# zengxianyu/sketchedit

Hardware: AMD Instinct MI355X
Metric: images/sec (higher is better)
Workload: dtype f32; 1 GPU; SketchEdit inference forward (netM+netG, use_cam, pool max) 256x256 batch 32 per GPU, procedural weights; global_batch=32, size=256, per_gpu_batch=32, execution=default, two streams

## Files before the change

### sketchedit_amd/_lib.py

```python
import contextlib
import ctypes
import os
import subprocess
import threading

import numpy as np

_HERE = os.path.dirname(os.path.abspath(__file__))
LIB_PATH = os.environ.get("SKETCHEDIT_HIP_LIB") or os.path.join(_HERE, "lib", "libsketchedit_hip.so")
CSRC = os.path.join(_HERE, "csrc")
SOURCES = ["se_gconv.hip", "se_rconv16.hip", "se_rconv96.hip", "se_rtile.hip", "se_rtilew.hip", "se_wino.hip", "se_wino24.hip", "se_wino48.hip", "se_wino_up.hip", "se_wino_up48.hip", "se_attention.hip", "se_att_stream.hip", "se_misc.hip", "se_resize.hip",
           "se_window.hip", "se_feather.hip", "se_fill.hip", "se_select.hip", "se_lasso.hip", "se_modify.hip", "se_outline.hip", "se_move.hip", "se_warp.hip", "se_filter.hip", "se_adjust.hip", "se_png.hip", "se_jpg.hip", "se_pack.hip",
           "se_plan.hip", "se_api_window.hip", "se_api_select.hip", "se_api_move.hip", "se_api_codec.hip", "se_api_debug.hip", "se_api.hip"]

SE_NET_G, SE_NET_M = 0, 1
RESAMPLE_LANCZOS, RESAMPLE_BILINEAR, RESAMPLE_BICUBIC = 1, 2, 3
FLAG_USE_CAM, FLAG_POOL_MAX, FLAG_NO_MASK_CC, FLAG_NO_MASK_COARSE, FLAG_JOINT_TRAIN_INP = 1, 2, 4, 8, 16
FLAG_LOW_LATENCY, FLAG_GRAPH, FLAG_PACKED_OUT, FLAG_BF16, FLAG_CONSERVATIVE = 32, 64, 128, 256, 512
LOW_LATENCY_MAX_PIXELS = 3 * 256 * 256
LOW_LATENCY_MAX_SINGLE_IMAGE = 512 * 512

SYMBOLS = ["se_create", "se_destroy", "se_last_error", "se_version", "se_load_weights", "se_weights_ready",
           "se_workspace_bytes", "se_netM_forward", "se_netM_forward_ex", "se_netG_forward", "se_netG_forward_taps", "se_inference", "se_inference_u8", "se_gated_conv2d",
           "se_gated_conv2d_ex", "se_attention", "se_attention_ex", "se_quantize_u8", "se_dequantize_u8", "se_inference_u8io", "se_profile_enable",
           "se_profile_report", "se_debug_set_option", "se_debug_get_option", "se_debug_reset_options", "se_debug_gconv_form",
           "se_resize_u8", "se_prepare_u8", "se_edit_u8", "se_edit_u8_workspace_bytes", "se_resample_coeffs",
# ... 317 lines not shown
    load_library().se_debug_reset_options()


def gconv_form(cin, cout, H, W, k=3, stride=1, rate=1, act="elu", upsample=False, cin1=0, x1_is_vector=False, B=1,
               low_latency=False, bf16=False, conservative=False, net=SE_NET_G):
    flags = (FLAG_LOW_LATENCY if low_latency else 0) | (FLAG_BF16 if bf16 else 0) | (FLAG_CONSERVATIVE if conservative else 0)
    buf = ctypes.create_string_buffer(64)
    fn = load_library().se_debug_gconv_form
    fn.argtypes, fn.restype = [ctypes.c_int] * 14 + [ctypes.c_char_p, ctypes.c_size_t], ctypes.c_int
    if fn(cin, cin1, int(bool(x1_is_vector)), cout, k, stride, rate, {"elu": 0, "relu": 1, None: 2}[act],
          int(bool(upsample)), B, H, W, flags, net, buf, len(buf)):
        raise SketchEditHipError("gconv_form: not a layer gated_conv2d takes")
    return buf.value.decode().split(",")


def pair_rule(B, H, W, low_latency=False):
    v = ctypes.c_int(-1)
    name = "SE_PAIR_RULE:%d,%d,%d,%d" % (B, H, W, FLAG_LOW_LATENCY if low_latency else 0)
    if load_library().se_debug_get_option(name.encode(), ctypes.byref(v)):
        raise SketchEditHipError("pair_rule: bad shape B=%d H=%d W=%d" % (B, H, W))
    return bool(v.value)


def flags_from_opt(opt):
    f = 0
    if getattr(opt, "use_cam", False):
        f |= FLAG_USE_CAM
    pool = getattr(opt, "pool_type", "avg")
    if pool == "max":
        f |= FLAG_POOL_MAX
# ... 1096 lines not shown
```

### sketchedit_amd/csrc/se_api_debug.hip

```cpp
#include "se_host.h"

using namespace se;

extern "C" {

int se_profile_enable(se_ctx* c, int on) {
  if (!c) return 1;
  std::lock_guard<std::mutex> lk(c->mu);
  HIPCHK(c, hipSetDevice(c->device));
  c->prof.recs.clear();
  c->prof.used = 0;
  if (on && c->prof.pool.empty()) {
    c->prof.pool.resize(2 * 1024);
    for (auto& e : c->prof.pool) HIPCHK(c, hipEventCreate(&e));
  }
  c->prof.on = on != 0;
  return 0;
}

int se_profile_report(se_ctx* c, char* buf, size_t cap) {
  if (!c || !buf || cap < 64) return 1;
  std::lock_guard<std::mutex> lk(c->mu);
  HIPCHK(c, hipSetDevice(c->device));
  HIPCHK(c, hipDeviceSynchronize());
// ... 44 lines not shown
    first = false;
  }
  s += "]}";
  if (s.size() + 1 > cap) return fail(c, "profile buffer too small");
  memcpy(buf, s.c_str(), s.size() + 1);
  return 0;
}

int se_debug_set_option(const char* name, int value) { return opt_set(name, value); }
int se_debug_get_option(const char* name, int* value) {
  static const char q[] = "SE_PAIR_RULE:";
  if (name && value && !strncmp(name, q, sizeof q - 1)) {
    int B = 0, H = 0, W = 0, flags = 0, end = 0;
    if (sscanf(name + sizeof q - 1, "%d,%d,%d,%d%n", &B, &H, &W, &flags, &end) != 4 || name[sizeof q - 1 + end] || B < 1 || H < 1 || W < 1) return 1;
    *value = pair_rule(B, H, W, flags) ? 1 : 0;
    return 0;
  }
  return opt_get(name, value);
}
void se_debug_reset_options(void) { opt_reset(); }

int se_debug_gconv_form(int cin, int cin1, int src1_is_vector, int cout, int k, int stride, int rate, int act, int upsample,
                        int B, int H, int W, int exec_flags, int net_id, char* out, size_t cap) {
  if (!out || cin <= 0 || cin1 < 0 || cout <= 0 || k <= 0 || stride <= 0 || rate <= 0 || B <= 0 || H <= 0 || W <= 0) return 1;
  const bool bf = (exec_flags & SE_FLAG_BF16) != 0;
  const int gran = bf ? 8 : 4;
  if (cin1 && ((cin % gran) || (cin1 % gran))) return 1;
  const LayerDef d = {"test", cin + cin1, cout, k, stride, rate, act, upsample};
  const bool raw = small_layer(d);
  if (raw && (k != 3 || cin != 12 || cin1 || (cout != 1 && cout != 3) || stride != 1 || rate != 1 || upsample)) return 1;
// ... 224 lines not shown
```

### sketchedit_amd/csrc/se_dispatch.h

```cpp
#pragma once
#include "se_kernels.h"

namespace se {

enum { ACT_ELU = 0, ACT_RELU = 1, ACT_NONE = 2 };

struct LayerDef {
  const char* name;
  int cin, cout, k, stride, rate, act, up;
};

inline bool small_layer(const LayerDef& d) { return d.act == ACT_NONE || d.cout == 3; }

struct ConvShape { int Ho, Wo, pad; };
inline ConvShape conv_shape(const LayerDef& d, int Hin, int Win) {
  const int pad = d.rate * (d.k - 1) / 2;
  if (d.up) return {2 * Hin, 2 * Win, pad};
  const int span = d.rate * (d.k - 1) + 1;
  return {(Hin + 2 * pad - span) / d.stride + 1, (Win + 2 * pad - span) / d.stride + 1, pad};
}

inline int choose_cfg(int G) {
  if (G <= 16) return GC_N24;
  if (G <= 24) return GC_N48;
// ... 3 lines not shown
}

inline bool rconv96_eligible(const LayerDef& d) {
  if (d.cout != 96 || d.rate != 1 || d.k != 3 || d.act == ACT_NONE) return false;
  if (d.stride == 2) return !d.up && d.cin == 24;
  if (d.stride != 1) return false;
  return d.up ? d.cin == 96 : (d.cin == 48 || d.cin == 24);
}

struct LayerFacts {
  bool small;
  int cfg, NP, G, T;
  int nch[2], CG[2];
  int dense, nchd;
  bool u, ub, u1, wv, wv16, u24, ub24, u24b, wx, wx2, wd, wdw, w16d, w16s, w96;
};

inline LayerFacts layer_facts(const LayerDef& d, int nchans) {
  LayerFacts f = {};
  f.cfg = -1;
  f.small = small_layer(d);
  if (f.small) return f;
  f.G = d.cout / 2;
  if (choose_cfg(f.G) < 0 || (f.G % 4)) return f;
  f.cfg = choose_cfg(f.G);
  f.NP = gconv_np(f.cfg);
  const int KW = d.up ? 2 : d.k;
  f.T = KW * KW;
  for (int bf = 0; bf < 2; ++bf) {
    const int per = bf ? 8 : 4, Cp = (nchans + per - 1) / per * per;
    f.CG[bf] = Cp / per;
    f.nch[bf] = (f.T * Cp + 8 * per - 1) / (8 * per);
  }
  const bool first = d.k == 5 && d.stride == 1 && d.rate == 1 && d.cout == 48;
  f.w16d = first && nchans >= 3 && nchans <= 4;
  f.wd = f.wdw = first && nchans >= 3 && nchans <= 5;
  f.dense = f.wd ? nchans : 0;
  f.nchd = (25 * f.dense + 31) / 32;
  f.w16s = d.k == 3 && d.stride == 1 && !d.up && (d.cin == 96 || d.cin == 192) && d.cout == 192;
  f.w96 = rconv96_eligible(d);
  if (d.k != 3 || d.stride != 1 || (nchans + 3) / 4 * 4 != d.cin) return f;
  if (d.up) {
    f.u = f.ub = (d.cin == 96 && d.cout == 96) || (d.cin == 48 && d.cout == 48);
  } else if ((d.cin == 96 || d.cin == 192) && d.cout == 192) {
    f.u = f.u24 = f.ub24 = true;
    f.u1 = f.wv = f.wv16 = f.u24b = d.cin == 192;
  } else if (d.cin == 48 && d.cout == 192) {
    f.u24 = f.ub24 = true;
  } else if (d.cin == 24 && d.cout == 24 && d.rate == 1) {
    f.wx = f.wx2 = true;
  } else if ((d.cin == 48 || d.cin == 24) && d.cout == 96) {
    f.u = f.ub = true;
  }
  return f;
}

enum { SRC2_NONE = 0, SRC2_TENSOR = 1, SRC2_VECTOR = 2 };
struct ConvCall {
  LayerDef def; LayerFacts facts;
  int B, Hin, Win, C0, C1;
  int src2;
  bool bf16, low_latency, conservative;
  int net;
  bool fold_scratch;
};

enum Form {
  F_SMALL_CONV, F_WINO, F_WINO24, F_WINO24_C48, F_WINO48, F_WINO48_C24, F_WINOUP, F_WINOUP48, F_RTILEW, F_RTILEW2,
  F_RTILE_DENSE5, F_RTILE_DENSE5W, F_RTILE_D4, F_RTILE, F_RCONV16, F_RCONV16_DUAL, F_RCONV96, F_GATHER
};
struct Choice {
  Form form;
  bool fold;
  bool wino_range;
};

inline bool magic_cg_ok(int CG, int nch) {
  const int m = (65536 + CG - 1) / CG;
  for (int gi = 0; gi < nch * 8 + 8; ++gi)
    if (((gi * m) >> 16) != gi / CG) return false;
  return true;
}
inline bool magic_kw_ok(int KW, int T) {
  const int m = 256 / KW + 1;
// ... 76 lines not shown
    const bool f43_net_ok = q.net == 0 || (f43_mode == 1 && !q.conservative);
    const bool f43 = (f43_mode == 1 || f43_mode == 2) && f43_net_ok && (s1 ? (!vec && f.u24b) : f.u24) && f.ub24 && (Win % (4 * d.rate)) == 0;
    return is(f43 ? F_WINO24 : F_WINO);
  }
  if (use_wino && f43_mode != 0 && !d.up && !two && C0 == 48 && d.cin == 48 && d.cout == 192 && d.stride == 1 && f.u24 && f.ub24 && fits96 &&
      (Hin % (2 * d.rate)) == 0 && (Win % (4 * d.rate)) == 0 && grid_ok(((long)(Hin / 2) * (Win / 4) + 31) / 32, min192))
    return is(F_WINO24_C48);
  if (use_wino && opt(OPT_WINOGRAD48) != 0 && !d.up && f.u && f.ub && !two && fits48 && even2 && grid_ok(wg64, min48)) {
    if (C0 == 48 && d.cin == 48) return is(F_WINO48);
    if (C0 == 24 && d.cin == 24 && d.cout == 96 && d.stride == 1) return is(F_WINO48_C24);
  }
  if (use_wino && opt(OPT_WINOGRAD_UP) != 0 && d.up && f.u && f.ub && !two && (Hin % 2) == 0 && (Win % 2) == 0 && grid_ok(4 * wg64, min48)) {
    if (C0 == 96 && d.cin == 96 && fits96) return is(F_WINOUP);
    if (opt(OPT_WINOGRAD_UP48) != 0 && C0 == 48 && d.cin == 48 && d.cout == 48 && fits48 && B * sh.Ho * sh.Wo * 96 < (1ll << 31)) return is(F_WINOUP48);
  }
  return is(choose_rtile(q));
}

inline const char* gconv_form_name(int cfg, bool small_grid, bool up2, bool two_src, bool bf16) {
#define SE_GF(n) n, n "_bf16", n "_2src", n "_2src_bf16", n "_up2", n "_up2_bf16", n "_up2_2src", n "_up2_2src_bf16"
#define SE_GS(n) { SE_GF(n), SE_GF(n "_small") }
  static const char* const names[4][16] = {SE_GS("gconv_n192"), SE_GS("gconv_n96"), SE_GS("gconv_n48"), SE_GS("gconv_n24")};
#undef SE_GS
#undef SE_GF
  if (cfg < 0 || cfg > 3) return nullptr;
  return names[cfg][(small_grid ? 8 : 0) | (up2 ? 4 : 0) | (two_src ? 2 : 0) | (bf16 ? 1 : 0)];
}

inline const char* form_name(const Choice& ch, const ConvCall& q) {
  const LayerDef& d = q.def;
// ... 3 lines not shown
    case F_WINO: return two ? "wino_2src" : "wino";
    case F_WINO24: return two ? "wino24_2src" : "wino24";
    case F_WINO24_C48: return "wino24_c48";
    case F_WINO48: return "wino48";
    case F_WINO48_C24: return "wino48_c24";
    case F_WINOUP: return "winoup";
    case F_WINOUP48: return "winoup48";
    case F_RTILEW: return "rtilew";
    case F_RTILEW2: return "rtilew2";
    case F_RTILE_DENSE5: return "rtile_dense5";
    case F_RTILE_DENSE5W: return "rtile_dense5w";
    case F_RTILE_D4: return "rtile_bf16_d4";
    case F_RTILE: return q.bf16 ? (d.up ? "rtile_bf16_up2" : "rtile_bf16") : (d.up ? "rtile_up2" : "rtile");
    case F_RCONV16: return "rconv16";
    case F_RCONV16_DUAL: return "rconv16_dual";
    case F_RCONV96: return d.up ? "rconv96_up" : d.stride == 2 ? "rconv96_s2" : q.C0 == 24 ? "rconv96_c24" : "rconv96";
    case F_GATHER: return gconv_form_name(q.facts.cfg, q.low_latency, d.up != 0, q.C0 / (q.bf16 ? 8 : 4) != q.facts.CG[q.bf16], q.bf16);
  }
  return nullptr;
}

}
```

### sketchedit_amd/csrc/se_kernels.h

```cpp
#pragma once
#include <hip/hip_runtime.h>
#include <stddef.h>
#include <stdint.h>

#include <vector>

struct se_window;

namespace se {

enum ProfLabel { PL_GCONV_N192 = 0, PL_GCONV_N96, PL_GCONV_N48, PL_GCONV_N24, PL_WINO_N192, PL_WINO_N96, PL_WINO_UP96, PL_SMALL_CONV, PL_PACK, PL_COLREDUCE,
                 PL_ATT_PREP, PL_ATT_SCORE, PL_ATT_SOFTMAX, PL_ATT_BOXSUM, PL_ATT_PV, PL_LAYOUT,
                 PL_ATT_STREAM_STATS, PL_ATT_STREAM_OUT, PL_RESIZE_H, PL_RESIZE_V, PL_WINDOW_GATHER, PL_WINDOW_BORDER, PL_WINDOW_PASTE,
                 PL_WINDOW_RESAMPLE_H, PL_WINDOW_PASTE_V, PL_WINDOW_SAVE, PL_WINDOW_SWAP, PL_WINDOW_LOCK_GATHER, PL_WINDOW_PASTE_LOCKED,
                 PL_WINDOW_PASTE_V_LOCKED, PL_SKETCH_TILES, PL_SKETCH_STROKES, PL_PNG_ROWS, PL_PNG_STRIPES,
                 PL_PNG_FINISH, PL_JPG_BLOCKS, PL_JPG_ROWS, PL_JPG_FINISH, PL_JPG2_BLOCKS, PL_JPG2_HIST, PL_JPG2_TABLES,
                 PL_WINDOW_PASTE_FEATHER, PL_FILL_MASKS, PL_FILL_KEEP, PL_SELECT_SIMILAR, PL_SELECT_FLOOD, PL_SELECT_GROW, PL_MODIFY_DISC, PL_MODIFY_VOTE,
                 PL_LASSO_FILL, PL_PLANE_COMBINE, PL_ADJUST, PL_HIST_TILES, PL_HIST_SUM, PL_ADJUST_LUT, PL_OUTLINE_COUNT, PL_OUTLINE_SCAN, PL_OUTLINE_EMIT, PL_FILTER_BLUR, PL_FILTER_MOSAIC, PL_MOVE_DROP,
                 PL_PLANE_SHIFT, PL_WARP_DROP, PL_PLANE_WARP, PL_COUNT };
const char* prof_label_name(int l);
struct Profiler {
  struct Rec { int label; const char* name; const char* form; double flops; double exec_flops; double bytes; long blocks; hipEvent_t a, b; };
  std::vector<Rec> recs;
  std::vector<hipEvent_t> pool;
// ... 5 lines not shown
void set_launch_grid(long blocks);
hipError_t ensure_max_lds(const void* func, int bytes);

#define SE_OPTIONS(X)                                                                                         \
  X(XCD_REMAP, 1)                                                             \
  X(RTILE, 1)                                              \
  X(RTILE_LL_MIN, 256)         \
  X(RTILE_WX, 2)          \
  X(RTILE_DENSE, 1)                                          \
  X(RTILE_D5W, 1)                                        \
  X(TEST_OFFSET_LIMIT, 0)  \
  X(TEST_POISON, 0)       \
  X(RCONV16, 1) X(RCONV16_DUAL, 1) X(RCONV96, 1) X(VECBIAS, 1)                                                  \
  X(WINOGRAD, 1) X(WINOGRAD48, 1) X(WINOGRAD_UP, 1) X(WINOGRAD_UP48, 1)                                         \
  X(WINOGRAD_F43, 1)      \
  X(GCONV_FAST, 1) X(FORK_DEFAULT, 1) X(LL_WINO_MIN_WG, 64) X(LL_WINO48_MIN_WG, 128)                            \
  X(ATT_FUSED, -1) X(ATT_FUSED_BF16, -1) X(ATT_PTILDE_LDS, 1) X(ATT_STATS_LDS, 1) X(ATT_E16, 1) X(ATT_SYM, 1)   \
  X(ATT_STREAM, 0)        \
  X(PAIR_MIN_PIXELS, 1 << 21)
enum Opt {
#define X(name, dflt) OPT_##name,
  SE_OPTIONS(X)
#undef X
  OPT_COUNT
};
int opt(int o);
int opt_set(const char* name, int value);
int opt_get(const char* name, int* value);
void opt_reset();
long long opt_epoch();
// ... 56 lines not shown
  int total_tiles;
  int act;
  int xcd;
  unsigned div_tpi_m, div_tw_m, div_d_m;
  int div_tpi_l, div_tw_l, div_d_l;
  const float* vbias;
};
hipError_t launch_wino(const WinoParams& p, hipStream_t st);
hipError_t launch_vecbias(const float* wv, const float* vec, float* T, int B, int C1, hipStream_t st, int round_vec = 0);
hipError_t launch_wino24(const WinoParams& p, hipStream_t st);
hipError_t launch_wino24_c48(const WinoParams& p, hipStream_t st);
hipError_t launch_wino48(const WinoParams& p, hipStream_t st);
hipError_t launch_wino48_c24(const WinoParams& p, hipStream_t st);
hipError_t launch_winoup(const WinoParams& p, hipStream_t st);
hipError_t launch_winoup48(const WinoParams& p, hipStream_t st);

struct RConvParams {
  const void* src;
  const void* wpk;
  const float* bias;
  void* dst;
  int B, h, w, d;
  int hs, ws;
  int ty, tx;
  int act;
  int xcd;
  const float* vbias;
  int dual;
};
hipError_t launch_rconv16(const RConvParams& p, hipStream_t st);
// ... 218 lines not shown
```

### sketchedit_amd/csrc/se_pack.h

```cpp
#pragma once
#include <hip/hip_runtime.h>

#include "se_dispatch.h"

#include <cstddef>
#include <string>
#include <vector>

namespace se {

class DevBuf {
 public:
  DevBuf() = default;
  DevBuf(const DevBuf&) = delete;
  DevBuf& operator=(const DevBuf&) = delete;
  DevBuf(DevBuf&& o) noexcept : p_(o.p_) { o.p_ = nullptr; }
  DevBuf& operator=(DevBuf&& o) noexcept {
    if (this != &o) { reset(); p_ = o.p_; o.p_ = nullptr; }
    return *this;
  }
  ~DevBuf() { reset(); }
  hipError_t alloc(size_t bytes) { reset(); return hipMalloc(&p_, bytes); }
  void reset() {
    if (p_) (void)hipFree(p_);
// ... 15 lines not shown
  DevBuf d_u;
  DevBuf d_ub;
  DevBuf d_w16d;
  DevBuf d_w16s;
  DevBuf d_w96;
  DevBuf d_u1;
  DevBuf d_wv;
  DevBuf d_wv16;
  DevBuf d_u24;
  DevBuf d_ub24;
  DevBuf d_u24b;
  DevBuf d_wx;
  DevBuf d_wx2;
  DevBuf d_wd;
  DevBuf d_wdw;
};

int pack_layer_images(Layer& L, const std::vector<int>& chans, std::string& err);

}
```

### sketchedit_amd/csrc/se_pack.hip

```cpp
#include "se_pack.h"
#include "se_kernels.h"

#include <cstring>

namespace se {
namespace {

template <class V>
int upload(DevBuf& dst, const std::vector<V>& host, std::string& err) {
  const size_t bytes = host.size() * sizeof(V);
  hipError_t e = dst.alloc(bytes);
  if (e == hipSuccess) e = hipMemcpy(dst, host.data(), bytes, hipMemcpyHostToDevice);
  if (e == hipSuccess) return 0;
  err = std::string("weight image upload failed: ") + hipGetErrorString(e);
  return 1;
}

unsigned short bf16_bits(float f) {
  unsigned u;
  memcpy(&u, &f, 4);
  if ((u & 0x7fffffffu) > 0x7f800000u) return (unsigned short)((u >> 16) | 0x40);
  u += 0x7fffu + ((u >> 16) & 1u);
  return (unsigned short)(u >> 16);
}
// ... 375 lines not shown
      const int oc = mixed_row_channel(n, 24);
      for (int ic = 0; ic < 48; ++ic) {
        float U[3][3];
        winoup_class(&L.w[((size_t)oc * d.cin + ic) * 9], cls >> 1, cls & 1, U);
        for (int pos = 0; pos < 9; ++pos) {
          const int pp = pos >> 1, u6 = (pos & 1) * 3 + ic / 16;
          const int it = pp * 3 + u6 / 2, kin = (u6 % 2) * 16 + ic % 16;
          img[(((size_t)cls * NIT + it) * NP + n) * 32 + swz(n, kin / 4, kin % 4)] = U[pos / 3][pos % 3];
        }
      }
    }
  if (upload(L.d_u, img, err)) return 1;
  return upload(L.d_ub, mixed_bias(L, NP), err);
}

int pack_small(Layer& L, std::string& err) {
  const LayerDef& d = L.def;
  std::vector<float> img((size_t)d.cout * 9 * 12);
  for (int oc = 0; oc < d.cout; ++oc)
    for (int t = 0; t < 9; ++t)
      for (int ic = 0; ic < 12; ++ic) img[((size_t)oc * 9 + t) * 12 + ic] = L.w[(((size_t)oc * 12 + ic) * 3 + t / 3) * 3 + t % 3];
  if (upload(L.direct[0], img, err) || upload(L.d_b, L.b, err)) return 1;
  for (auto& v : img) v = bf16_round(v);
  if (upload(L.direct[1], img, err)) return 1;
  L.packed = true;
  return 0;
}

int pack_gated(Layer& L, const std::vector<int>& chans, std::string& err) {
  const LayerFacts& f = L.facts;
  const int nc = (int)chans.size();
  auto padded = [&](int per) {
    std::vector<int> m(chans);
    m.resize((nc + per - 1) / per * per, -1);
    return m;
  };
  if (pack_direct<unsigned short>(L, padded(8), err)) return 1;
  if (f.w16d && pack_layer16_d4(L, padded(4), err)) return 1;
  if (f.w16s && pack_rconv16(L, err)) return 1;
  if (f.w96 && pack_rconv96(L, err)) return 1;
  if (f.wd && pack_layer_dense(L, chans, err)) return 1;
  return pack_layer(L, padded(4), err);
}

}

int pack_layer_images(Layer& L, const std::vector<int>& chans, std::string& err) {
  const LayerFacts f = L.facts = layer_facts(L.def, (int)chans.size());
  if (f.small ? pack_small(L, err) : pack_gated(L, chans, err)) return 1;
  const struct { const char* name; const float* img; bool fact; } have[] = {
      {"u", L.d_u, f.u}, {"ub", L.d_ub, f.ub}, {"u1", L.d_u1, f.u1}, {"wv", L.d_wv, f.wv}, {"wv16", L.d_wv16, f.wv16},
      {"u24", L.d_u24, f.u24}, {"ub24", L.d_ub24, f.ub24}, {"u24b", L.d_u24b, f.u24b}, {"wx", L.d_wx, f.wx}, {"wx2", L.d_wx2, f.wx2},
      {"wd", L.d_wd, f.wd}, {"wdw", L.d_wdw, f.wdw}, {"w16d", L.d_w16d, f.w16d}, {"w16s", L.d_w16s, f.w16s}, {"w96", L.d_w96, f.w96}};
  for (const auto& h : have)
    if ((h.img != nullptr) != h.fact) {
      err = std::string("layer ") + L.def.name + ": weight image " + h.name + (h.fact ? " is missing" : " was built against the layer's facts");
      return 1;
    }
  return 0;
}

}
```

### sketchedit_amd/csrc/se_plan.hip

```cpp
#include "se_host.h"

#include <numeric>

using namespace se;

namespace {

#define ENC(p)                                                                                    \
  {p "2_downsample", 24, 96, 3, 2, 1, ACT_ELU, 0}, {p "3", 48, 96, 3, 1, 1, ACT_ELU, 0},          \
      {p "4_downsample", 48, 192, 3, 2, 1, ACT_ELU, 0}, {p "5", 96, 192, 3, 1, 1, ACT_ELU, 0},    \
      {p "6", 96, 192, 3, 1, 1, ACT_ELU, 0}, {p "7_atrous", 96, 192, 3, 1, 2, ACT_ELU, 0},        \
      {p "8_atrous", 96, 192, 3, 1, 4, ACT_ELU, 0}, {p "9_atrous", 96, 192, 3, 1, 8, ACT_ELU, 0}, \
      {p "10_atrous", 96, 192, 3, 1, 16, ACT_ELU, 0}
#define DEC(p, c11in, c17out)                                                                        \
  {p "11", c11in, 192, 3, 1, 1, ACT_ELU, 0}, {p "12", 96, 192, 3, 1, 1, ACT_ELU, 0},                 \
      {p "13_upsample_conv", 96, 96, 3, 1, 1, ACT_ELU, 1}, {p "14", 48, 96, 3, 1, 1, ACT_ELU, 0},    \
      {p "15_upsample_conv", 48, 48, 3, 1, 1, ACT_ELU, 1}, {p "16", 24, 24, 3, 1, 1, ACT_ELU, 0},    \
      {p "17", 12, c17out, 3, 1, 1, ACT_NONE, 0}

}

namespace se {

const LayerDef G_LAYERS[] = {
// ... 54 lines not shown
    const float* s1 = folded ? nullptr : src1;
    WinoParams wp = f43 ? wino_params(s1 ? L.d_u24b : L.d_u24, L.d_ub24, d.rate, 4) : wino_params(folded ? L.d_u1 : L.d_u, L.d_b, d.rate, 2);
    wp.src1 = s1; wp.src1_vec = folded ? 0 : src1_vec; wp.vbias = folded ? c->vbias_ws : nullptr;
    if ((double)B * Hin * Win * 384.0 >= 2147483648.0) return fail(c, "layer %s: tensor exceeds 2^31 bytes", d.name);
    set_launch_cost(alg3x3, 4.0 * 2.0 * (double)B * Hin * Win * 96, d.name,
                    f43 ? alg3x3 * 24.0 / 72.0 * (folded ? 0.5 : 1.0) : alg3x3 * 16.0 / 36.0 * (folded ? 0.5 : 1.0));
    HIPCHK(c, f43 ? launch_wino24(wp, c->st) : launch_wino(wp, c->st));
    return 0;
  }
  int launch_form_wino48(const Choice& ch) const {
    const WinoParams wp = wino_params(L.d_u, L.d_ub, d.rate, 2);
    const bool c24 = ch.form == F_WINO48_C24;
    set_launch_cost(alg(9), c24 ? 4.0 * ((double)B * Hin * Win * 24 + (double)B * Hin * Win * 48) : 4.0 * 2.0 * (double)B * Hin * Win * 48, d.name,
                    alg(9) * 16.0 / 36.0);
    HIPCHK(c, c24 ? launch_wino48_c24(wp, c->st) : launch_wino48(wp, c->st));
    return 0;
  }
  int launch_form_winoup(const Choice& ch) const {
    const WinoParams wp = wino_params(L.d_u, L.d_ub, 1, 2);
    if (ch.form == F_WINOUP) {
      set_launch_cost(alg(9), 4.0 * ((double)B * Hin * Win * 96 + (double)B * Ho * Wo * 48), d.name, alg(9) * 9.0 / 36.0);
      HIPCHK(c, launch_winoup(wp, c->st));
      return 0;
    }
    set_launch_cost(alg(9), 4.0 * ((double)B * Hin * Win * 48 + (double)B * Ho * Wo * 24), d.name, alg(9) * 9.0 / 36.0 * 28.0 / 27.0);
    HIPCHK(c, launch_winoup48(wp, c->st));
    return 0;
  }

  RTileParams rtile_params(const float* wpk, int trows) const {
// ... 138 lines not shown
  if (ch.wino_range && !said) {
    said = true;
    fprintf(stderr, "sketchedit_hip: layer %s: %d x %dx%d x 96 floats exceed the Winograd kernel's 32-bit byte offsets; "
                    "using the direct kernel (about 2x slower) -- split the batch\n", d.name, B, Hin, Win);
  }
  const ConvLaunch a = {c, L, d, f, src0, C0, src1, C1, src1_vec, dst, B, Hin, Win, sh.Ho, sh.Wo, sh.pad, bf};
  switch (ch.form) {
    case F_WINO: case F_WINO24: case F_WINO24_C48: return a.launch_form_wino(ch);
    case F_WINO48: case F_WINO48_C24: return a.launch_form_wino48(ch);
    case F_WINOUP: case F_WINOUP48: return a.launch_form_winoup(ch);
    case F_RTILEW: case F_RTILEW2: return a.launch_form_rtilew(ch);
    case F_RTILE_DENSE5: case F_RTILE_DENSE5W: return a.launch_form_rtile_dense5(ch);
    case F_RTILE: case F_RTILE_D4: return a.launch_form_rtile(ch);
    case F_RCONV16: case F_RCONV16_DUAL: return a.launch_form_rconv16(ch);
    case F_RCONV96: return a.launch_form_rconv96(ch);
    case F_GATHER: return a.launch_form_gather(ch);
    case F_SMALL_CONV: break;
  }
  return fail(c, "layer %s: not a gated conv", d.name);
}

}

namespace {

Act encoder(Plan& P, const std::string& p, Act& in, Act* keep9, Layer* first = nullptr) {
  Act x = first ? P.conv_layer(*first, in) : P.conv((p + "1").c_str(), in);
  x = P.conv((p + "2_downsample").c_str(), x);
  x = P.conv((p + "3").c_str(), x);
  x = P.conv((p + "4_downsample").c_str(), x);
// ... 326 lines not shown
```

### sketchedit_amd/kernel_labels.py

```python

KERNEL_LABELS = {
    "wino_kernel": "wino_n192", "wino24_kernel": "wino_n192", "rconv16": "gconv_n192", "gconv_kernel<12": "gconv_n192",
    "wino48_kernel": "wino_n96", "rconv96": "gconv_n96", "gconv_kernel<6": "gconv_n96",
    "winoup_kernel": "wino_up96",
    "winoup48_kernel": "gconv_n48", "rtile_dense5w_kernel": "gconv_n48", "rtile_dense5_kernel": "gconv_n48",
    "rtile_kernel<3": "gconv_n48", "gconv_kernel<3": "gconv_n48",
    "rtilew2_kernel": "gconv_n24", "rtilew_kernel": "gconv_n24", "rtile_kernel<2": "gconv_n24", "gconv_kernel<2": "gconv_n24",
    "dtail_kernel": "dtail",
    "att2_pair_kernel": "att_score", "att2_pv_kernel": "att_pv",
    "att2_softmax": "att_softmax", "att2_stats": "att_softmax",
    "att2_boxsum": "att_boxsum", "att2_ptilde": "att_boxsum",
    "att2_prep": "att_prep", "att2_transpose": "att_prep", "att2_emean": "att_prep", "att2_eoff": "att_prep",
    "att2_similar": "layout",
    "small_conv_kernel": "small_conv", "pack_": "pack", "colreduce": "colreduce", "vecbias_kernel": "colreduce",
    "nchw_to_nhwc": "layout", "nhwc_to_nchw": "layout", "nhwc16_to_nchw": "layout", "quantize_u8_kernel": "layout",
    "dequant_u8_kernel": "layout",
    "(anonymous namespace)::window_resample_h_kernel": "window_resample_h", "(anonymous namespace)::window_paste_v_kernel": "window_paste_v",
    "window_resample_h_kernel": "window_resample_h", "window_paste_v_kernel": "window_paste_v",
    "(anonymous namespace)::resample_h_kernel": "resize_h", "(anonymous namespace)::resample_v_kernel": "resize_v",
    "resample_h_kernel": "resize_h", "resample_v_kernel": "resize_v",
    "(anonymous namespace)::window_gather_kernel": "window_gather", "(anonymous namespace)::window_border_kernel": "window_border",
    "(anonymous namespace)::window_paste_kernel": "window_paste",
    "window_gather_kernel": "window_gather", "window_border_kernel": "window_border", "window_paste_kernel": "window_paste",
    "(anonymous namespace)::window_paste_feather_kernel": "window_paste_feather", "window_paste_feather_kernel": "window_paste_feather",
# ... 49 lines not shown
```

Baseline: 3004 images/sec.

## Add polyphase Winograd-style kernel for stride-2 48-channel gated convolutions

Adds a new s2poly48 kernel for the 3x3 stride-2 gated convolutions with 48 input channels and 96 or 192 outputs. It splits each 4x4 input tile into polyphase components, transforms the filter into 25 combined positions, and runs the products on MFMA with triple-buffered LDS staging. The signed partial sums are then folded into 2x2 outputs. The intent is fewer multiplies and better data reuse than the generic rtile path, at the cost of extra packed weight images, more register pressure, and a new form that is on by default.

```diff
diff --git a/sketchedit_amd/_lib.py b/sketchedit_amd/_lib.py
--- a/sketchedit_amd/_lib.py
+++ b/sketchedit_amd/_lib.py
@@ -9,7 +9,7 @@
 _HERE = os.path.dirname(os.path.abspath(__file__))
 LIB_PATH = os.environ.get("SKETCHEDIT_HIP_LIB") or os.path.join(_HERE, "lib", "libsketchedit_hip.so")
 CSRC = os.path.join(_HERE, "csrc")
-SOURCES = ["se_gconv.hip", "se_rconv16.hip", "se_rconv96.hip", "se_rtile.hip", "se_rtilew.hip", "se_wino.hip", "se_wino24.hip", "se_wino48.hip", "se_wino_up.hip", "se_wino_up48.hip", "se_attention.hip", "se_att_stream.hip", "se_misc.hip", "se_resize.hip",
+SOURCES = ["se_gconv.hip", "se_rconv16.hip", "se_rconv96.hip", "se_rtile.hip", "se_rtilew.hip", "se_wino.hip", "se_wino24.hip", "se_wino48.hip", "se_wino_up.hip", "se_wino_up48.hip", "se_s2poly.hip", "se_attention.hip", "se_att_stream.hip", "se_misc.hip", "se_resize.hip",
            "se_window.hip", "se_feather.hip", "se_fill.hip", "se_select.hip", "se_lasso.hip", "se_modify.hip", "se_outline.hip", "se_move.hip", "se_warp.hip", "se_filter.hip", "se_adjust.hip", "se_png.hip", "se_jpg.hip", "se_pack.hip",
            "se_plan.hip", "se_api_window.hip", "se_api_select.hip", "se_api_move.hip", "se_api_codec.hip", "se_api_debug.hip", "se_api.hip"]
 
@@ -357,6 +357,28 @@
     return buf.value.decode().split(",")
 
 
+def s2poly_tables():
+    return np.array([[get_option("SE_S2POLY_TABLE:%d,%d" % (q, j)) for j in range(7)] for q in range(5)], np.int32)
+
+
+def s2poly_probe_layer(cout):
+    p = lambda n: (((7919 * n) % 2053 - 1026) / 1024.0).astype(np.float32)
+    return p(np.arange(cout * 48 * 9, dtype=np.int64)).reshape(cout, 48, 3, 3), p(10007 + np.arange(cout, dtype=np.int64))
+
+
+def s2poly_probe_pack(cout):
+    fn = load_library().se_debug_get_option
+    n = (cout // 96) * 38 * 96 * 32
+    out = np.zeros(n + cout, np.int32)
+    v = ctypes.c_int(0)
+    for i in range(n + cout):
+        if fn(("SE_S2POLY_PACK:%d,%d" % (cout, i)).encode(), ctypes.byref(v)):
+            raise SketchEditHipError("SE_S2POLY_PACK: cout must be 96 or 192")
+        out[i] = v.value
+    f = out.view(np.float32)
+    return f[:n].reshape(cout // 96, 38, 96, 32).copy(), f[n:].copy()
+
+
 def pair_rule(B, H, W, low_latency=False):
     v = ctypes.c_int(-1)
     name = "SE_PAIR_RULE:%d,%d,%d,%d" % (B, H, W, FLAG_LOW_LATENCY if low_latency else 0)
diff --git a/sketchedit_amd/csrc/se_api_debug.hip b/sketchedit_amd/csrc/se_api_debug.hip
--- a/sketchedit_amd/csrc/se_api_debug.hip
+++ b/sketchedit_amd/csrc/se_api_debug.hip
@@ -1,4 +1,5 @@
 #include "se_host.h"
+#include "se_s2poly.h"
 
 using namespace se;
 
@@ -82,6 +83,33 @@
     int B = 0, H = 0, W = 0, flags = 0, end = 0;
     if (sscanf(name + sizeof q - 1, "%d,%d,%d,%d%n", &B, &H, &W, &flags, &end) != 4 || name[sizeof q - 1 + end] || B < 1 || H < 1 || W < 1) return 1;
     *value = pair_rule(B, H, W, flags) ? 1 : 0;
+    return 0;
+  }
+  static const char qt[] = "SE_S2POLY_TABLE:", qp[] = "SE_S2POLY_PACK:";
+  if (name && value && !strncmp(name, qt, sizeof qt - 1)) {
+    int q = -1, j = -1, end = 0;
+    if (sscanf(name + sizeof qt - 1, "%d,%d%n", &q, &j, &end) != 2 || name[sizeof qt - 1 + end] || q < 0 || q > 4 || j < 0 || j > 6) return 1;
+    *value = j == 0 ? s2poly_src_a(q) : j == 1 ? s2poly_src_b(q) : j < 5 ? s2poly_wcoef(q, j - 2) : s2poly_fold(q, j - 5);
+    return 0;
+  }
+  if (name && value && !strncmp(name, qp, sizeof qp - 1)) {
+    int cout = 0, end = 0;
+    long long i = -1;
+    if (sscanf(name + sizeof qp - 1, "%d,%lld%n", &cout, &i, &end) != 2 || name[sizeof qp - 1 + end] || (cout != 96 && cout != 192) || i < 0) return 1;
+    static std::mutex mu;
+    static std::vector<float> kept[2];
+    std::lock_guard<std::mutex> lk(mu);
+    std::vector<float>& all = kept[cout == 192];
+    if (all.empty()) {
+      auto probe = [](long long n) { return (float)((7919 * n) % 2053 - 1026) / 1024.f; };
+      std::vector<float> w((size_t)cout * 48 * 9), b(cout), bias;
+      for (size_t n = 0; n < w.size(); ++n) w[n] = probe((long long)n);
+      for (int n = 0; n < cout; ++n) b[n] = probe(10007 + n);
+      if (!s2poly_pack_host(w.data(), b.data(), cout, all, bias)) return 1;
+      all.insert(all.end(), bias.begin(), bias.end());
+    }
+    if ((size_t)i >= all.size()) return 1;
+    memcpy(value, &all[(size_t)i], sizeof(int));
     return 0;
   }
   return opt_get(name, value);
diff --git a/sketchedit_amd/csrc/se_dispatch.h b/sketchedit_amd/csrc/se_dispatch.h
--- a/sketchedit_amd/csrc/se_dispatch.h
+++ b/sketchedit_amd/csrc/se_dispatch.h
@@ -41,6 +41,7 @@
   int nch[2], CG[2];
   int dense, nchd;
   bool u, ub, u1, wv, wv16, u24, ub24, u24b, wx, wx2, wd, wdw, w16d, w16s, w96;
+  bool s2p;
 };
 
 inline LayerFacts layer_facts(const LayerDef& d, int nchans) {
@@ -66,6 +67,7 @@
   f.nchd = (25 * f.dense + 31) / 32;
   f.w16s = d.k == 3 && d.stride == 1 && !d.up && (d.cin == 96 || d.cin == 192) && d.cout == 192;
   f.w96 = rconv96_eligible(d);
+  f.s2p = d.k == 3 && d.stride == 2 && d.rate == 1 && !d.up && nchans == 48 && d.cin == 48 && (d.cout == 96 || d.cout == 192);
   if (d.k != 3 || d.stride != 1 || (nchans + 3) / 4 * 4 != d.cin) return f;
   if (d.up) {
     f.u = f.ub = (d.cin == 96 && d.cout == 96) || (d.cin == 48 && d.cout == 48);
@@ -94,7 +96,7 @@
 
 enum Form {
   F_SMALL_CONV, F_WINO, F_WINO24, F_WINO24_C48, F_WINO48, F_WINO48_C24, F_WINOUP, F_WINOUP48, F_RTILEW, F_RTILEW2,
-  F_RTILE_DENSE5, F_RTILE_DENSE5W, F_RTILE_D4, F_RTILE, F_RCONV16, F_RCONV16_DUAL, F_RCONV96, F_GATHER
+  F_RTILE_DENSE5, F_RTILE_DENSE5W, F_RTILE_D4, F_RTILE, F_RCONV16, F_RCONV16_DUAL, F_RCONV96, F_S2POLY48, F_GATHER
 };
 struct Choice {
   Form form;
@@ -201,6 +203,10 @@
     if (C0 == 96 && d.cin == 96 && fits96) return is(F_WINOUP);
     if (opt(OPT_WINOGRAD_UP48) != 0 && C0 == 48 && d.cin == 48 && d.cout == 48 && fits48 && B * sh.Ho * sh.Wo * 96 < (1ll << 31)) return is(F_WINOUP48);
   }
+  const int s2_mode = opt(OPT_S2_POLY);
+  if ((s2_mode == 1 || (s2_mode == 2 && q.net == 0)) && !ll && f.s2p && !two && d.k == 3 && d.stride == 2 && d.rate == 1 && !d.up && C0 == 48 &&
+      d.cin == 48 && (d.cout == 96 || d.cout == 192) && (Hin % 4) == 0 && (Win % 4) == 0 && fits48)
+    return is(F_S2POLY48);
   return is(choose_rtile(q));
 }
 
@@ -234,6 +240,7 @@
     case F_RTILE: return q.bf16 ? (d.up ? "rtile_bf16_up2" : "rtile_bf16") : (d.up ? "rtile_up2" : "rtile");
     case F_RCONV16: return "rconv16";
     case F_RCONV16_DUAL: return "rconv16_dual";
+    case F_S2POLY48: return "s2poly48";
     case F_RCONV96: return d.up ? "rconv96_up" : d.stride == 2 ? "rconv96_s2" : q.C0 == 24 ? "rconv96_c24" : "rconv96";
     case F_GATHER: return gconv_form_name(q.facts.cfg, q.low_latency, d.up != 0, q.C0 / (q.bf16 ? 8 : 4) != q.facts.CG[q.bf16], q.bf16);
   }
diff --git a/sketchedit_amd/csrc/se_kernels.h b/sketchedit_amd/csrc/se_kernels.h
--- a/sketchedit_amd/csrc/se_kernels.h
+++ b/sketchedit_amd/csrc/se_kernels.h
@@ -43,6 +43,7 @@
   X(RCONV16, 1) X(RCONV16_DUAL, 1) X(RCONV96, 1) X(VECBIAS, 1)                                                  \
   X(WINOGRAD, 1) X(WINOGRAD48, 1) X(WINOGRAD_UP, 1) X(WINOGRAD_UP48, 1)                                         \
   X(WINOGRAD_F43, 1)      \
+  X(S2_POLY, 1)           \
   X(GCONV_FAST, 1) X(FORK_DEFAULT, 1) X(LL_WINO_MIN_WG, 64) X(LL_WINO48_MIN_WG, 128)                            \
   X(ATT_FUSED, -1) X(ATT_FUSED_BF16, -1) X(ATT_PTILDE_LDS, 1) X(ATT_STATS_LDS, 1) X(ATT_E16, 1) X(ATT_SYM, 1)   \
   X(ATT_STREAM, 0)        \
@@ -129,6 +130,7 @@
 hipError_t launch_wino48_c24(const WinoParams& p, hipStream_t st);
 hipError_t launch_winoup(const WinoParams& p, hipStream_t st);
 hipError_t launch_winoup48(const WinoParams& p, hipStream_t st);
+hipError_t launch_s2poly48(const WinoParams& p, int halves, hipStream_t st);
 
 struct RConvParams {
   const void* src;
diff --git a/sketchedit_amd/csrc/se_pack.h b/sketchedit_amd/csrc/se_pack.h
--- a/sketchedit_amd/csrc/se_pack.h
+++ b/sketchedit_amd/csrc/se_pack.h
@@ -53,6 +53,8 @@
   DevBuf d_wx2;
   DevBuf d_wd;
   DevBuf d_wdw;
+  DevBuf d_s2p;
+  DevBuf d_s2pb;
 };
 
 int pack_layer_images(Layer& L, const std::vector<int>& chans, std::string& err);
diff --git a/sketchedit_amd/csrc/se_pack.hip b/sketchedit_amd/csrc/se_pack.hip
--- a/sketchedit_amd/csrc/se_pack.hip
+++ b/sketchedit_amd/csrc/se_pack.hip
@@ -1,5 +1,6 @@
 #include "se_pack.h"
 #include "se_kernels.h"
+#include "se_s2poly.h"
 
 #include <cstring>
 
@@ -413,6 +414,17 @@
   return upload(L.d_ub, mixed_bias(L, NP), err);
 }
 
+int pack_s2poly48(Layer& L, std::string& err) {
+  const LayerDef& d = L.def;
+  std::vector<float> img, bias;
+  if (d.cin != 48 || (int)L.w.size() != d.cout * 48 * 9 || !s2poly_pack_host(L.w.data(), L.b.data(), d.cout, img, bias)) {
+    err = std::string("layer ") + d.name + ": no polyphase image for this shape";
+    return 1;
+  }
+  if (upload(L.d_s2p, img, err)) return 1;
+  return upload(L.d_s2pb, bias, err);
+}
+
 int pack_small(Layer& L, std::string& err) {
   const LayerDef& d = L.def;
   std::vector<float> img((size_t)d.cout * 9 * 12);
@@ -439,6 +451,11 @@
   if (f.w16s && pack_rconv16(L, err)) return 1;
   if (f.w96 && pack_rconv96(L, err)) return 1;
   if (f.wd && pack_layer_dense(L, chans, err)) return 1;
+  if (f.s2p) {
+    for (int i = 0; i < nc; ++i)
+      if (chans[i] != i) { err = std::string("layer ") + L.def.name + ": the polyphase image needs its input channels in checkpoint order"; return 1; }
+    if (pack_s2poly48(L, err)) return 1;
+  }
   return pack_layer(L, padded(4), err);
 }
 
@@ -450,7 +467,8 @@
   const struct { const char* name; const float* img; bool fact; } have[] = {
       {"u", L.d_u, f.u}, {"ub", L.d_ub, f.ub}, {"u1", L.d_u1, f.u1}, {"wv", L.d_wv, f.wv}, {"wv16", L.d_wv16, f.wv16},
       {"u24", L.d_u24, f.u24}, {"ub24", L.d_ub24, f.ub24}, {"u24b", L.d_u24b, f.u24b}, {"wx", L.d_wx, f.wx}, {"wx2", L.d_wx2, f.wx2},
-      {"wd", L.d_wd, f.wd}, {"wdw", L.d_wdw, f.wdw}, {"w16d", L.d_w16d, f.w16d}, {"w16s", L.d_w16s, f.w16s}, {"w96", L.d_w96, f.w96}};
+      {"wd", L.d_wd, f.wd}, {"wdw", L.d_wdw, f.wdw}, {"w16d", L.d_w16d, f.w16d}, {"w16s", L.d_w16s, f.w16s}, {"w96", L.d_w96, f.w96},
+      {"s2p", L.d_s2p, f.s2p}, {"s2pb", L.d_s2pb, f.s2p}};
   for (const auto& h : have)
     if ((h.img != nullptr) != h.fact) {
       err = std::string("layer ") + L.def.name + ": weight image " + h.name + (h.fact ? " is missing" : " was built against the layer's facts");
diff --git a/sketchedit_amd/csrc/se_plan.hip b/sketchedit_amd/csrc/se_plan.hip
--- a/sketchedit_amd/csrc/se_plan.hip
+++ b/sketchedit_amd/csrc/se_plan.hip
@@ -92,6 +92,16 @@
     set_launch_cost(alg(9), c24 ? 4.0 * ((double)B * Hin * Win * 24 + (double)B * Hin * Win * 48) : 4.0 * 2.0 * (double)B * Hin * Win * 48, d.name,
                     alg(9) * 16.0 / 36.0);
     HIPCHK(c, c24 ? launch_wino48_c24(wp, c->st) : launch_wino48(wp, c->st));
+    return 0;
+  }
+  int launch_form_s2poly(const Choice&) const {
+    const int halves = d.cout / 96;
+    WinoParams wp = wino_params(L.d_s2p, L.d_s2pb, 1, 2);
+    wp.th = Hin / 4; wp.tw = Win / 4; wp.total_tiles = B * wp.th * wp.tw;
+    udiv_magic_host((unsigned)(wp.th * wp.tw), &wp.div_tpi_m, &wp.div_tpi_l);
+    udiv_magic_host((unsigned)wp.tw, &wp.div_tw_m, &wp.div_tw_l);
+    set_launch_cost(alg(9), 4.0 * ((double)halves * B * Hin * Win * 48 + (double)B * Ho * Wo * (d.cout / 2)), d.name, alg(9) * 25.0 / 36.0);
+    HIPCHK(c, launch_s2poly48(wp, halves, c->st));
     return 0;
   }
   int launch_form_winoup(const Choice& ch) const {
@@ -260,6 +270,7 @@
     case F_RTILE: case F_RTILE_D4: return a.launch_form_rtile(ch);
     case F_RCONV16: case F_RCONV16_DUAL: return a.launch_form_rconv16(ch);
     case F_RCONV96: return a.launch_form_rconv96(ch);
+    case F_S2POLY48: return a.launch_form_s2poly(ch);
     case F_GATHER: return a.launch_form_gather(ch);
     case F_SMALL_CONV: break;
   }
diff --git a/sketchedit_amd/csrc/se_s2poly.h b/sketchedit_amd/csrc/se_s2poly.h
--- /dev/null
+++ b/sketchedit_amd/csrc/se_s2poly.h
@@ -0,0 +1,45 @@
+#pragma once
+#include <hip/hip_runtime.h>
+
+#include <cstddef>
+#include <vector>
+
+namespace se {
+
+constexpr int S2POLY_NPOS = 25;
+constexpr int S2POLY_NIT = 38;
+
+__host__ __device__ constexpr int s2poly_src_a(int q) { return q == 0 ? 1 : q == 1 ? 3 : q == 2 ? 0 : 2; }
+__host__ __device__ constexpr int s2poly_src_b(int q) { return q == 2 ? 2 : q == 4 ? 4 : -1; }
+__host__ __device__ constexpr int s2poly_wcoef(int q, int k) { return q < 2 ? k == 1 : q == 2 ? k == 0 : q == 3 ? k != 1 : k == 2; }
+__host__ __device__ constexpr int s2poly_fold(int q, int o) {
+  return o == 0 ? (q == 0 || q == 2 || q == 3 ? 1 : 0) : (q == 1 || q == 3 ? 1 : q == 4 ? -1 : 0);
+}
+
+inline bool s2poly_pack_host(const float* w, const float* b, int cout, std::vector<float>& img, std::vector<float>& bias) {
+  if (cout != 96 && cout != 192) return false;
+  const int NP = cout, G = cout / 2;
+  img.assign((size_t)(NP / 96) * S2POLY_NIT * 96 * 32, 0.f);
+  bias.assign((size_t)NP, 0.f);
+  for (int n = 0; n < NP; ++n) {
+    const int f = n / 16 * 8 + n % 8, oc = n % 16 < 8 ? f : G + f;
+    const int hf = n / 96, r = n % 96;
+    bias[n] = b[oc];
+    for (int ic = 0; ic < 48; ++ic) {
+      const float* g = w + ((size_t)oc * 48 + ic) * 9;
+      for (int pos = 0; pos < S2POLY_NPOS; ++pos) {
+        const int py = pos / 5, px = pos % 5;
+        double u = 0.;
+        for (int ky = 0; ky < 3; ++ky)
+          for (int kx = 0; kx < 3; ++kx) u += (double)(s2poly_wcoef(py, ky) * s2poly_wcoef(px, kx)) * (double)g[ky * 3 + kx];
+        const int pp = pos >> 1, u6 = (pos & 1) * 3 + ic / 16;
+        const int it = pp * 3 + u6 / 2, kin = (u6 % 2) * 16 + ic % 16;
+        const int slot = (kin / 4) ^ ((r >> 1) & 7);
+        img[(((size_t)hf * S2POLY_NIT + it) * 96 + r) * 32 + slot * 4 + kin % 4] = (float)u;
+      }
+    }
+  }
+  return true;
+}
+
+}
diff --git a/sketchedit_amd/csrc/se_s2poly.hip b/sketchedit_amd/csrc/se_s2poly.hip
--- /dev/null
+++ b/sketchedit_amd/csrc/se_s2poly.hip
@@ -0,0 +1,298 @@
+#include "se_device.h"
+#include "se_s2poly.h"
+
+#include <cstdlib>
+#include <type_traits>
+
+namespace se {
+
+template <int I, int N, typename F>
+DEVFN void static_for_s2(F&& f) {
+  if constexpr (I < N) {
+    f(std::integral_constant<int, I>{});
+    static_for_s2<I + 1, N>(f);
+  }
+}
+
+__global__ __launch_bounds__(256, 2) void s2poly48_kernel(const WinoParams p) {
+  constexpr int TILES = 64, NTHR = 256, NWV = 4;
+  constexpr int XB = TILES * 128, WB = 96 * 128;
+  constexpr int NPOS = S2POLY_NPOS, NIT = S2POLY_NIT;
+  constexpr unsigned PSB = 192;
+  extern __shared__ __attribute__((aligned(16))) char smem[];
+  char* Xb = smem;
+  char* Wb = smem + 3 * XB;
+
+  const int tid = threadIdx.x, lane = tid & 63;
+  const float eluw = p.act == 0 ? 1.f : 0.f;
+  const int w = __builtin_amdgcn_readfirstlane(tid >> 6);
+  const int chh = w & 1, tp = w >> 1;
+  const int half = (int)blockIdx.y;
+  const int tile_base = (p.xcd ? xcd_tile(blockIdx.x, gridDim.x) : (int)blockIdx.x) * TILES;
+  const int tpi = p.th * p.tw;
+  const float* upk = p.upk + (size_t)half * NIT * 96 * 32;
+  const float* bias = p.bias + half * 96;
+
+  auto tile_origin = [&](int t, int& b, int& iy, int& ix) {
+    b = (int)udiv_magic((unsigned)t, p.div_tpi_m, p.div_tpi_l);
+    const int rem = t - b * tpi;
+    iy = (int)udiv_magic((unsigned)rem, p.div_tw_m, p.div_tw_l);
+    ix = rem - iy * p.tw;
+  };
+
+  const int sg = tid & 3, srow = (tid >> 6) * 16 + ((tid >> 2) & 1) * 8 + ((tid >> 3) & 7);
+  const int swz = (srow >> 1) & 7;
+  char* xw0 = Xb + srow * 128 + ((sg ^ swz) << 4);
+  char* xw1 = Xb + srow * 128 + (((4 + sg) ^ swz) << 4);
+  int* Ysrc = (int*)(smem + 3 * XB + 4 * WB);
+  int* Xsrc = Ysrc + 5 * NTHR;
+  {
+    const int t = tile_base + srow;
+    int b, iy, ix;
+    tile_origin(t < p.total_tiles ? t : 0, b, iy, ix);
+#pragma unroll
+    for (int i = 0; i < 5; ++i) {
+      const int y = 4 * iy - 1 + i;
+      Ysrc[i * NTHR + tid] = (t < p.total_tiles && (unsigned)y < (unsigned)p.h) ? (int)((unsigned)((b * p.h + y) * p.w) * PSB + (unsigned)sg * 16u) : (int)(0x80000000u + (unsigned)sg * 16u);
+    }
+    if (tid < TILES) {
+      const int t2 = tile_base + tid;
+      tile_origin(t2 < p.total_tiles ? t2 : 0, b, iy, ix);
+#pragma unroll
+      for (int i = 0; i < 5; ++i) {
+        const int x = 4 * ix - 1 + i;
+        Xsrc[i * TILES + tid] = ((unsigned)x < (unsigned)p.w) ? x * (int)PSB : (int)0x80000000;
+      }
+    }
+  }
+  __syncthreads();
+  const unsigned lds_w = lds_addr_of(Wb);
+  int off0, off1;
+  frag_offsets(lane, off0, off1);
+
+  auto need = [&](int pos, int i) {
+    if (pos >= NPOS) return false;
+    return !((i >= 2 && s2poly_src_b(pos / 5) < 0) || ((i & 1) && s2poly_src_b(pos % 5) < 0));
+  };
+  unsigned o[2][4];
+  auto set_pos = [&](int set, int pos) {
+    const int py = pos / 5, px = pos % 5;
+    const unsigned ya = (unsigned)Ysrc[s2poly_src_a(py) * NTHR + tid], xa = (unsigned)Xsrc[s2poly_src_a(px) * TILES + srow];
+    o[set][0] = __builtin_elementwise_add_sat(ya, xa);
+    if (s2poly_src_b(px) >= 0) o[set][1] = __builtin_elementwise_add_sat(ya, (unsigned)Xsrc[s2poly_src_b(px) * TILES + srow]);
+    if (s2poly_src_b(py) >= 0) {
+      const unsigned yb = (unsigned)Ysrc[s2poly_src_b(py) * NTHR + tid];
+      o[set][2] = __builtin_elementwise_add_sat(yb, xa);
+      if (s2poly_src_b(px) >= 0) o[set][3] = __builtin_elementwise_add_sat(yb, (unsigned)Xsrc[s2poly_src_b(px) * TILES + srow]);
+    }
+  };
+  auto half_set = [](int it, int h) { return (it % 3) * 2 + h >= 3 ? 1 : 0; };
+  auto half_grp = [](int it, int h) { return ((it % 3) * 2 + h) % 3; };
+  auto half_pos = [&](int it, int h) { return 2 * (it / 3) + half_set(it, h); };
+  const __amdgpu_buffer_rsrc_t rs0 = __builtin_amdgcn_make_buffer_rsrc((void*)p.src, 0, (int)((unsigned)p.B * (unsigned)p.h * (unsigned)p.w * PSB), 0x00020000);
+  auto load_x1 = [&](int it, f32x4 (&r)[2][4], int h, int i) {
+    typedef unsigned u32x4 __attribute__((ext_vector_type(4)));
+    if (need(half_pos(it, h), i))
+      r[h][i] = __builtin_bit_cast(f32x4, (u32x4)__builtin_amdgcn_raw_buffer_load_b128(rs0, (int)o[half_set(it, h)][i], half_grp(it, h) * 64, 0));
+  };
+  float negone = -1.f;
+  asm volatile("" : "+v"(negone));
+  auto signed_sum = [&](const f32x4 (&q)[4], int pos) -> f32x4 {
+    f32x4 ps = q[0], ns = {0.f, 0.f, 0.f, 0.f};
+    bool hn = false;
+    if (need(pos, 3)) ps = ps + q[3];
+#pragma unroll
+    for (int i = 1; i < 3; ++i)
+      if (need(pos, i)) { ns = hn ? ns + q[i] : q[i]; hn = true; }
+    return hn ? ns * negone + ps : ps;
+  };
+  auto write_x = [&](int it, int buf, const f32x4 (&r)[2][4]) {
+    *(f32x4*)(xw0 + buf * XB) = signed_sum(r[0], half_pos(it, 0));
+    if (half_pos(it, 1) < NPOS) *(f32x4*)(xw1 + buf * XB) = signed_sum(r[1], half_pos(it, 1));
+  };
+  auto dma_w = [&](int it, int buf, int j) {
+    const int rbk = j * NWV + w;
+    glds16_s(upk + (size_t)it * 96 * 32 + rbk * 256, (unsigned)lane * 16u, lds_w + buf * WB + rbk * 1024);
+  };
+
+  f32x4 am[3][2];
+  f32x4 oy[2][2][3][2];
+#pragma unroll
+  for (int j = 0; j < 3; ++j)
+#pragma unroll
+    for (int q = 0; q < 2; ++q) {
+      am[j][q] = (f32x4){0.f, 0.f, 0.f, 0.f};
+      const f32x4 b4 = *(const f32x4*)(bias + (3 * chh + j) * 16 + (lane >> 4) * 4);
+#pragma unroll
+      for (int a = 0; a < 2; ++a)
+#pragma unroll
+        for (int b = 0; b < 2; ++b) oy[a][b][j][q] = b4;
+    }
+  float neg1 = -1.f;
+  asm volatile("" : "+v"(neg1));
+  auto fold = [&](int pos) {
+    const int py = pos / 5, px = pos % 5;
+    const int ay[2] = {s2poly_fold(py, 0), s2poly_fold(py, 1)};
+    const int ax[2] = {s2poly_fold(px, 0), s2poly_fold(px, 1)};
+#pragma unroll
+    for (int j = 0; j < 3; ++j)
+#pragma unroll
+      for (int q = 0; q < 2; ++q) {
+#pragma unroll
+        for (int a = 0; a < 2; ++a)
+#pragma unroll
+          for (int b = 0; b < 2; ++b) {
+            const int c = ay[a] * ax[b];
+            if (c > 0) oy[a][b][j][q] += am[j][q];
+            else if (c < 0) oy[a][b][j][q] = am[j][q] * neg1 + oy[a][b][j][q];
+          }
+        asm volatile("" : "+v"(oy[0][0][j][q]), "+v"(oy[0][1][j][q]), "+v"(oy[1][0][j][q]), "+v"(oy[1][1][j][q]));
+      }
+  };
+
+  auto end_barrier = [&]() {
+    __builtin_amdgcn_sched_barrier(0);
+    asm volatile("s_waitcnt lgkmcnt(0)\n\ts_barrier" ::: "memory");
+    __builtin_amdgcn_sched_barrier(0);
+  };
+
+  f32x4 r[2][4];
+  set_pos(0, 0);
+  set_pos(1, 1);
+#pragma unroll
+  for (int i0 = 0; i0 < 3; ++i0) { dma_w(i0, i0, 0); dma_w(i0, i0, 1); dma_w(i0, i0, 2); }
+  {
+    f32x4 r1[2][4];
+#pragma unroll
+    for (int i = 0; i < 4; ++i) { load_x1(0, r, 0, i); load_x1(0, r, 1, i); }
+#pragma unroll
+    for (int i = 0; i < 4; ++i) { load_x1(1, r1, 0, i); load_x1(1, r1, 1, i); }
+    write_x(0, 0, r);
+    write_x(1, 1, r1);
+  }
+  set_pos(0, 2);
+  dma_wait_all();
+  __syncthreads();
+#pragma unroll
+  for (int i = 0; i < 4; ++i) { load_x1(2, r, 0, i); load_x1(2, r, 1, i); }
+
+  const char* Xw = Xb + tp * 32 * 128;
+  const char* Ww = Wb + (3 * chh) * 2048;
+  f32x4 wa[3], xa[2];
+  xa[0] = *(const f32x4*)(Xw + off0);
+  xa[1] = *(const f32x4*)(Xw + 2048 + off0);
+#pragma unroll
+  for (int j = 0; j < 3; ++j) wa[j] = *(const f32x4*)(Ww + j * 2048 + off0);
+
+  static_for_s2<0, NIT>([&](auto it_c) __attribute__((always_inline)) {
+    constexpr int it = decltype(it_c)::value;
+    constexpr int pp = it / 3, c = it % 3;
+    constexpr int b0 = it % 3, b1 = (it + 1) % 3, b2 = (it + 2) % 3;
+    constexpr int w0 = it % 4, w1 = (it + 1) % 4, w3 = (it + 3) % 4;
+    constexpr bool more1 = it + 1 < NIT, more2 = it + 2 < NIT, more3 = it + 3 < NIT;
+    constexpr bool second = 2 * pp + (c >= 1 ? 1 : 0) < NPOS;
+    f32x4 wb[3], xb[2];
+    if (second) {
+      xb[0] = *(const f32x4*)(Xw + b0 * XB + off1);
+      xb[1] = *(const f32x4*)(Xw + b0 * XB + 2048 + off1);
+#pragma unroll
+      for (int j = 0; j < 3; ++j) wb[j] = *(const f32x4*)(Ww + w0 * WB + j * 2048 + off1);
+    }
+    __builtin_amdgcn_sched_barrier(0);
+    auto group = [&](const f32x4 (&wf)[3], const f32x4 (&xf)[2], int e, bool first) {
+#pragma unroll
+      for (int j = 0; j < 3; ++j)
+#pragma unroll
+        for (int q = 0; q < 2; ++q) {
+          const f32x4 cin = first ? (f32x4){0.f, 0.f, 0.f, 0.f} : am[j][q];
+          am[j][q] = __builtin_amdgcn_mfma_f32_16x16x4f32(wf[j][e], xf[q][e], cin, 0, 0, 0);
+        }
+      __builtin_amdgcn_sched_barrier(0);
+    };
+    if (c == 0 && it > 0) {
+      fold(2 * pp - 1);
+      __builtin_amdgcn_sched_barrier(0);
+    }
+    group(wa, xa, 0, c == 0);
+    group(wa, xa, 1, false);
+    group(wa, xa, 2, false);
+    group(wa, xa, 3, false);
+    if (c == 1) {
+      fold(2 * pp);
+      __builtin_amdgcn_sched_barrier(0);
+    }
+    if (more2) {
+      dma_wait_all();
+      write_x(it + 2, b2, r);
+    }
+    if (c == 2 && 2 * (pp + 2) < NPOS) set_pos(0, 2 * (pp + 2));
+    if (c == 0 && 2 * (pp + 1) + 1 < NPOS) set_pos(1, 2 * (pp + 1) + 1);
+    __builtin_amdgcn_sched_barrier(0);
+    if (second) group(wb, xb, 0, c == 1);
+    if (more3) { dma_w(it + 3, w3, 0); load_x1(it + 3, r, 0, 0); load_x1(it + 3, r, 0, 1); }
+    if (more1) {
+      xa[0] = *(const f32x4*)(Xw + b1 * XB + off0);
+      xa[1] = *(const f32x4*)(Xw + b1 * XB + 2048 + off0);
+#pragma unroll
+      for (int j = 0; j < 3; ++j) wa[j] = *(const f32x4*)(Ww + w1 * WB + j * 2048 + off0);
+    }
+    __builtin_amdgcn_sched_barrier(0);
+    if (second) group(wb, xb, 1, false);
+    if (more3) { dma_w(it + 3, w3, 1); load_x1(it + 3, r, 0, 2); load_x1(it + 3, r, 0, 3); }
+    __builtin_amdgcn_sched_barrier(0);
+    if (second) group(wb, xb, 2, false);
+    if (more3) { dma_w(it + 3, w3, 2); load_x1(it + 3, r, 1, 0); load_x1(it + 3, r, 1, 1); }
+    __builtin_amdgcn_sched_barrier(0);
+    if (second) group(wb, xb, 3, false);
+    if (more3) { load_x1(it + 3, r, 1, 2); load_x1(it + 3, r, 1, 3); }
+    if (more1) end_barrier();
+  });
+
+  const int q = lane >> 4;
+  const int OH = p.h >> 1, OW = p.w >> 1;
+  const unsigned pix_bytes = 192u * gridDim.y;
+#pragma unroll
+  for (int tq = 0; tq < 2; ++tq) {
+    const int t = tile_base + tp * 32 + tq * 16 + (lane & 15);
+    int b = 0, iy = 0, ix = 0;
+    tile_origin(t < p.total_tiles ? t : 0, b, iy, ix);
+#pragma unroll
+    for (int j = 0; j < 3; ++j) {
+      const int c0 = half * 48 + (3 * chh + j) * 8 + (q & 1) * 4 + (q >> 1) * 2;
+#pragma unroll
+      for (int a = 0; a < 2; ++a)
+#pragma unroll
+        for (int bb = 0; bb < 2; ++bb) {
+          const f32x4 v = oy[a][bb][j][tq];
+          const auto s02 = __builtin_amdgcn_permlane32_swap(__float_as_uint(v[0]), __float_as_uint(v[2]), false, false);
+          const auto s13 = __builtin_amdgcn_permlane32_swap(__float_as_uint(v[1]), __float_as_uint(v[3]), false, false);
+          const float f0 = __uint_as_float(s02[0]), g0 = __uint_as_float(s02[1]);
+          const float f1 = __uint_as_float(s13[0]), g1 = __uint_as_float(s13[1]);
+          float2 ov;
+          ov.x = act_fast(f0, eluw) * sigmoid_fast(g0);
+          ov.y = act_fast(f1, eluw) * sigmoid_fast(g1);
+          if (t < p.total_tiles)
+            *(float2*)((char*)p.dst + ((unsigned)((b * OH + 2 * iy + a) * OW + 2 * ix + bb) * pix_bytes + (unsigned)c0 * 4u)) = ov;
+        }
+    }
+  }
+}
+
+hipError_t launch_s2poly48(const WinoParams& p, int halves, hipStream_t st) {
+  constexpr int TILES = 64;
+  constexpr int LDS = 3 * TILES * 128 + 4 * 96 * 128 + 5 * TILES * 4 * 4 + 5 * TILES * 4;
+  static_assert(LDS <= 80 * 1024, "two workgroups per CU");
+  if ((halves != 1 && halves != 2) || (p.h % 4) || (p.w % 4) || p.th != p.h / 4 || p.tw != p.w / 4) return hipErrorInvalidValue;
+  if ((double)p.B * p.h * p.w * 192.0 >= 2147483648.0) return hipErrorInvalidValue;
+  {
+    hipError_t e = ensure_max_lds((const void*)s2poly48_kernel, LDS);
+    if (e != hipSuccess) return e;
+  }
+  const int grid = (p.total_tiles + TILES - 1) / TILES;
+  set_launch_grid((long)grid * halves);
+  ProfScope ps_(st, PL_WINO_N96, "s2poly48");
+  hipLaunchKernelGGL(s2poly48_kernel, dim3(grid, halves), dim3(TILES * 4), LDS, st, p);
+  return hipGetLastError();
+}
+
+}
diff --git a/sketchedit_amd/kernel_labels.py b/sketchedit_amd/kernel_labels.py
--- a/sketchedit_amd/kernel_labels.py
+++ b/sketchedit_amd/kernel_labels.py
@@ -2,6 +2,7 @@
 KERNEL_LABELS = {
     "wino_kernel": "wino_n192", "wino24_kernel": "wino_n192", "rconv16": "gconv_n192", "gconv_kernel<12": "gconv_n192",
     "wino48_kernel": "wino_n96", "rconv96": "gconv_n96", "gconv_kernel<6": "gconv_n96",
+    "s2poly48_kernel": "wino_n96",
     "winoup_kernel": "wino_up96",
     "winoup48_kernel": "gconv_n48", "rtile_dense5w_kernel": "gconv_n48", "rtile_dense5_kernel": "gconv_n48",
     "rtile_kernel<3": "gconv_n48", "gconv_kernel<3": "gconv_n48",
```

Result: faster. 3055 images/sec (median of 6 runs) (+1.7%).
